# ShittyWizard/DiplomJourney

Hardware: NVIDIA B200
Metric: candidate rollouts/s (MPC inner loop) (higher is better)
Workload: dtype f32

## Files before the change

### diplomjourney_b200/build.py

```python
from __future__ import annotations

import hashlib
import os
import shutil
import subprocess
import sys

HERE = os.path.dirname(os.path.abspath(__file__))
CSRC = os.path.join(HERE, "csrc")
LIB = os.environ.get("MPCB_LIB") or os.path.join(HERE, "lib", "libmpcb200.so")
SOURCES = ["mpcb_kernels.cu", "mpcb_loop.cu", "mpcb_api.cu", "mpcb_nccl.cu"]
HEADERS = ["mpcb_types.cuh", "mpcb_bounds.cuh", "mpcb_exact.cuh", "mpcb_handle.cuh", "mpcb_events.cuh", "mpcb_noise.cuh", "mpcb_pcg64.cuh", "mpcb_screen.cuh", os.path.join("..", "..", "include", "mpcb200.h")]
NVCC_FLAGS = [
    "-gencode", "arch=compute_100a,code=sm_100a", "-O3", "-lineinfo", "-std=c++17",
    "-Xcompiler", "-fPIC", "-Xcompiler", "-fvisibility=hidden", "--shared",
]


def _nvcc() -> str:
    for cand in (os.environ.get("NVCC"), shutil.which("nvcc"), "/usr/local/cuda/bin/nvcc"):
        if cand and os.path.exists(cand):
            return cand
    raise RuntimeError("nvcc not found: the CUDA library cannot be built (there is no CPU fallback)")


def source_hash() -> str:
    h = hashlib.sha256(" ".join(NVCC_FLAGS).encode())
    for name in SOURCES + HEADERS:
        with open(os.path.join(CSRC, name), "rb") as f:
            h.update(name.encode() + b"\0" + f.read())
    return h.hexdigest()


def needs_build(lib: str | None = None) -> bool:
    lib = lib or LIB
    try:
        with open(lib + ".srchash") as f:
            return not os.path.exists(lib) or f.read().strip() != source_hash()
    except OSError:
        return True


def build_library(force: bool = False, verbose: bool = False, extra_flags=(), out: str | None = None) -> str:
    out = out or LIB
    if not force and out == LIB and (os.environ.get("MPCB_LIB") or not needs_build()):
        if not os.path.exists(LIB):
            raise RuntimeError(f"MPCB_LIB={LIB} does not exist")
        return LIB
    os.makedirs(os.path.dirname(out), exist_ok=True)
    cmd = [_nvcc()] + NVCC_FLAGS + list(extra_flags) + (["-Xptxas", "-v"] if verbose else []) + \
          [os.path.join(CSRC, s) for s in SOURCES] + ["-o", out, "-ldl"]
    r = subprocess.run(cmd, capture_output=True, text=True)
    if r.returncode != 0:
        raise RuntimeError("nvcc failed:\n" + r.stdout + r.stderr)
    if not extra_flags:
        with open(out + ".srchash", "w") as f:
            f.write(source_hash() + "\n")
    if verbose:
        print(r.stderr)
    return out


if __name__ == "__main__":
    print(build_library(force="--force" in sys.argv, verbose="-v" in sys.argv))
```

### diplomjourney_b200/csrc/mpcb_api.cu

```cuda
#include "../../include/mpcb200.h"
#include "mpcb_types.cuh"
#include "mpcb_bounds.cuh"
#include "mpcb_handle.cuh"
#include "mpcb_noise.cuh"
#include "mpcb_pcg64.cuh"

#include <algorithm>
#include <cmath>
#include <cstdarg>
#include <cstdio>
#include <cstring>
#include <string>
#include <vector>

namespace mpcb {
cudaError_t launch_prep(cudaStream_t, long long, const double *, const double *, const double *, const double *,
                        const uint8_t *, int, int, int, double, double, double, SolveParams *);
cudaError_t launch_pass(cudaStream_t, const LaunchArgs &, const RowPairs &, int pass, bool prefix, int sms);
cudaError_t launch_reduce_compact(cudaStream_t, const LaunchArgs &, double *, unsigned *, unsigned *, int sms);
cudaError_t launch_reduce_compact_wide(cudaStream_t, const LaunchArgs &, double *, unsigned *, unsigned *, void *scratch,
                                       int sms, int *launches);
cudaError_t launch_probe(cudaStream_t, const LaunchArgs &, int sms);
cudaError_t launch_tilecut(cudaStream_t, const LaunchArgs &, unsigned long long g_begin, unsigned long long g_end,
                           unsigned long long *list, unsigned *count, unsigned long long list_cap);
cudaError_t launch_frontier_expand(cudaStream_t, const LaunchArgs &, int k, const unsigned long long *src,
                                   const unsigned *src_count, unsigned long long *dst, unsigned *dst_count,
                                   unsigned *overflow, int sms);
cudaError_t launch_tilewalk_fallback(cudaStream_t, const LaunchArgs &, unsigned long long all_tiles, int sms);
cudaError_t launch_cand_resolve(cudaStream_t, const LaunchArgs &, int sms);
cudaError_t launch_refine_scan(cudaStream_t, const LaunchArgs &, int sms);
cudaError_t launch_finalize(cudaStream_t, const LaunchArgs &, double *, long long *, double *, double *);
cudaError_t launch_dump(cudaStream_t, const LaunchArgs &, bool prefix, double *jrel, int sms);
cudaError_t launch_held_loop(cudaStream_t, const LoopArgs &, int sms);
cudaError_t launch_rng_seed(cudaStream_t, long long N, const unsigned *keys, int key_len, unsigned *rng_state);
cudaError_t launch_pcg64_seed(cudaStream_t, long long N, const unsigned *entropy, int ent_len, int ent_stride,
                              const unsigned *spawn, int spawn_len, unsigned long long *pcg_state);
cudaError_t launch_held_small(cudaStream_t, const SmallArgs &);
cudaError_t launch_full_apply(cudaStream_t, const FullLoopArgs &);
cudaError_t launch_held_windows(cudaStream_t, const WindowArgs &, int sms);
cudaError_t launch_split_ub_min(cudaStream_t, const LaunchArgs &, const unsigned long long *all, int nranks);
cudaError_t launch_split_pack(cudaStream_t, const LaunchArgs &, SplitRec *mine);
cudaError_t launch_split_pick(cudaStream_t, const LaunchArgs &, const SplitRec *all, int nranks);
bool nccl_available();
int nccl_comm_info(void *comm, int *nranks, int *rank);
int nccl_allgather_bytes(void *comm, const void *send, void *recv, size_t bytes, cudaStream_t st);
}

using namespace mpcb;

namespace {

int fail(mpcb_handle *h, int code, const char *fmt, ...) {
    char buf[512];
    va_list ap;
    va_start(ap, fmt);
// ... 102 lines not shown
    std::vector<float2> c32(S), c32s(S);
    double vmin_grid = v[0];
    for (int i = 1; i < nv; ++i) vmin_grid = std::min(vmin_grid, v[i]);
    const double v_slow = vmin_grid > v_min ? vmin_grid : v_min;
    double smax = 0, dphimax = 0, smin = INFINITY;
    for (int iv = 0; iv < nv; ++iv)
        for (int ib = 0; ib < nb; ++ib) {
            const int c = iv * nb + ib;
            for (int variant = 0; variant < 2; ++variant) {
                const double vc = variant ? v_slow : v[iv];
                const double dphi = (vc / L) * std::tan(beta[ib]) * delta_t;
                const double s = vc * delta_t;
                const double cd = std::cos(dphi), sd = std::sin(dphi);
                smax = std::max(smax, std::fabs(s));
                smin = std::min(smin, s);
                dphimax = std::max(dphimax, std::fabs(dphi));
                if (variant == 0) {
                    t64[c] = make_double4(cd, sd, s, dphi);
                    vt[c] = vc;
                    l32[c] = make_float4((float)(s * cd), (float)(s * sd), (float)(s * s),
                                         (float)(3.16227766016837952 * dphi));
                    c32[c] = make_float2((float)dphi, (float)s);
                } else {
                    t64s[c] = make_double4(cd, sd, s, dphi);
                    vts[c] = vc;
                    c32s[c] = make_float2((float)dphi, (float)s);
                }
            }
        }
    std::vector<float4> t32(S);
    for (int c = 0; c < S; ++c) t32[c] = make_float4((float)t64[c].x, (float)t64[c].y, (float)t64[c].z, (float)t64[c].w);
    CK(h->tab32.ensure(sizeof(float4) * S));
    CK(h->tab64.ensure(sizeof(double4) * S)); CK(h->tab64_slow.ensure(sizeof(double4) * S));
    CK(h->vtab.ensure(sizeof(double) * S)); CK(h->vtab_slow.ensure(sizeof(double) * S));
    CK(h->beta.ensure(sizeof(double) * nb));
    const int npairs = (S + 1) / 2;
    std::vector<float4> l32p(2 * (size_t)npairs);
    for (int m = 0; m < npairs; ++m) {
        const float4 x = l32[2 * m], y = l32[std::min(2 * m + 1, S - 1)];
        l32p[2 * m] = make_float4(x.x, y.x, x.y, y.y);
        l32p[2 * m + 1] = make_float4(x.z, y.z, x.w, y.w);
    }
    const int ppr = (nb + 1) / 2;
    const bool rows_fit = 2LL * nv * ppr <= kLeafChunk;
    std::vector<float4> l32r(rows_fit ? 2 * (size_t)nv * ppr : 0);
    if (rows_fit)
        for (int iv = 0; iv < nv; ++iv)
            for (int m = 0; m < ppr; ++m) {
                const float4 x = l32[iv * nb + 2 * m], y = l32[iv * nb + std::min(2 * m + 1, nb - 1)];
                l32r[2 * ((size_t)iv * ppr + m)] = make_float4(x.x, y.x, x.y, y.y);
                l32r[2 * ((size_t)iv * ppr + m) + 1] = make_float4(x.z, y.z, x.w, y.w);
                h->row_ab.ab[iv * ppr + m] = l32r[2 * ((size_t)iv * ppr + m)];
            }
    CK(h->leaf32r.ensure(sizeof(float4) * std::max<size_t>(l32r.size(), 1)));
    CK(h->leaf32.ensure(sizeof(float4) * S));
    CK(h->leaf32p.ensure(sizeof(float4) * 2 * npairs));
    CK(h->ctl32.ensure(sizeof(float2) * S)); CK(h->ctl32_slow.ensure(sizeof(float2) * S));
    CK(cudaMemcpyAsync(h->tab64.p, t64.data(), sizeof(double4) * S, cudaMemcpyHostToDevice, h->stream));
    CK(cudaMemcpyAsync(h->tab32.p, t32.data(), sizeof(float4) * S, cudaMemcpyHostToDevice, h->stream));
    CK(cudaMemcpyAsync(h->tab64_slow.p, t64s.data(), sizeof(double4) * S, cudaMemcpyHostToDevice, h->stream));
    CK(cudaMemcpyAsync(h->vtab.p, vt.data(), sizeof(double) * S, cudaMemcpyHostToDevice, h->stream));
    CK(cudaMemcpyAsync(h->vtab_slow.p, vts.data(), sizeof(double) * S, cudaMemcpyHostToDevice, h->stream));
    CK(cudaMemcpyAsync(h->beta.p, beta, sizeof(double) * nb, cudaMemcpyHostToDevice, h->stream));
    CK(cudaMemcpyAsync(h->leaf32.p, l32.data(), sizeof(float4) * S, cudaMemcpyHostToDevice, h->stream));
    CK(cudaMemcpyAsync(h->leaf32p.p, l32p.data(), sizeof(float4) * 2 * npairs, cudaMemcpyHostToDevice, h->stream));
    if (rows_fit) CK(cudaMemcpyAsync(h->leaf32r.p, l32r.data(), sizeof(float4) * l32r.size(), cudaMemcpyHostToDevice, h->stream));
    CK(cudaMemcpyAsync(h->ctl32.p, c32.data(), sizeof(float2) * S, cudaMemcpyHostToDevice, h->stream));
    CK(cudaMemcpyAsync(h->ctl32_slow.p, c32s.data(), sizeof(float2) * S, cudaMemcpyHostToDevice, h->stream));
    GridTables &g = h->g;
    g.tab64 = h->tab64.as<double4>(); g.vtab = h->vtab.as<double>();
    g.tab32 = h->tab32.as<float4>();
    g.tab64_slow = h->tab64_slow.as<double4>(); g.vtab_slow = h->vtab_slow.as<double>();
    g.beta = h->beta.as<double>();
    g.leaf32 = h->leaf32.as<float4>();
    g.leaf32p = h->leaf32p.as<float4>();
    g.leaf32r = rows_fit ? h->leaf32r.as<float4>() : nullptr;
    g.nv = nv; g.ppr = rows_fit ? ppr : 0;
    g.ctl32 = h->ctl32.as<float2>(); g.ctl32_slow = h->ctl32_slow.as<float2>();
    g.S = S; g.nb = nb; g.dt = delta_t; g.smax = smax; g.dphimax = dphimax; g.smin = smin;
    g.sbox = ScreenBox{l32[0].x, l32[0].x, l32[0].y, l32[0].y, l32[0].w, l32[0].w};
    for (int c = 1; c < S; ++c) {
        g.sbox.amin = std::min(g.sbox.amin, l32[c].x); g.sbox.amax = std::max(g.sbox.amax, l32[c].x);
        g.sbox.bmin = std::min(g.sbox.bmin, l32[c].y); g.sbox.bmax = std::max(g.sbox.bmax, l32[c].y);
        g.sbox.gmin = std::min(g.sbox.gmin, l32[c].w); g.sbox.gmax = std::max(g.sbox.gmax, l32[c].w);
    }
    h->tables_ready = true;
    return MPCB_OK;
}


extern "C" {

int mpcb_version(void) { return 100; }

int mpcb_device_count(void) {
    int n = 0;
    if (cudaGetDeviceCount(&n) != cudaSuccess) return 0;
    return n;
}

int mpcb_create(int device_ordinal, mpcb_handle **out) {
    if (!out) return MPCB_ERR_INVALID;
    *out = nullptr;
    int n = 0;
    if (cudaGetDeviceCount(&n) != cudaSuccess || n <= 0) return MPCB_ERR_NO_DEVICE;
    if (device_ordinal < 0 || device_ordinal >= n) return MPCB_ERR_INVALID;
    mpcb_handle *h = new mpcb_handle_s();
    h->device = device_ordinal;
    if (cudaSetDevice(device_ordinal) != cudaSuccess ||
        cudaStreamCreateWithFlags(&h->stream, cudaStreamNonBlocking) != cudaSuccess) {
        delete h;
        return MPCB_ERR_CUDA;
    }
    cudaDeviceGetAttribute(&h->sms, cudaDevAttrMultiProcessorCount, device_ordinal);
    *out = h;
    return MPCB_OK;
}

int mpcb_destroy(mpcb_handle *h) {
    if (!h) return MPCB_OK;
    cudaSetDevice(h->device);
    cudaStreamSynchronize(h->stream);
    for (DevBuf *b : {&h->tab64, &h->tab32, &h->vtab, &h->tab64_slow, &h->vtab_slow, &h->beta, &h->leaf32, &h->leaf32p, &h->leaf32r, &h->ctl32,
                      &h->ctl32_slow, &h->sp, &h->segmin, &h->worklist, &h->misc, &h->tau, &h->bestJ, &h->bestIdx,
                      &h->lock, &h->ub, &h->tile_list, &h->reduce_scratch, &h->in_state, &h->in_target, &h->in_origin, &h->in_thr, &h->in_flags, &h->out_cost,
                      &h->out_index, &h->out_traj, &h->out_ctl, &h->dump_rec, &h->dump_j, &h->loop_log, &h->loop_ticks,
                      &h->loop_status, &h->loop_events, &h->loop_final, &h->loop_rng, &h->loop_keys, &h->small_in, &h->small_out, &h->fl_last, &h->fl_k, &h->fl_have, &h->fl_flags,
                      &h->fl_count, &h->nccl_scratch, &h->cand, &h->cand_J, &h->cand_sel, &h->node_list})
        b->release();
    if (h->pin_in) cudaFreeHost(h->pin_in);
    if (h->pin_out) cudaFreeHost(h->pin_out);
    cudaStreamDestroy(h->stream);
    delete h;
    return MPCB_OK;
}

const char *mpcb_last_error(const mpcb_handle *h) { return h ? h->err.c_str() : "null handle"; }
void *mpcb_stream(mpcb_handle *h) { return h ? (void *)h->stream : nullptr; }

int mpcb_sync(mpcb_handle *h) {
    if (!h) return MPCB_ERR_INVALID;
    CK(cudaSetDevice(h->device));
    CK(cudaStreamSynchronize(h->stream));
    return MPCB_OK;
}

int mpcb_set_option(mpcb_handle *h, const char *name, double value) {
    if (!h || !name) return MPCB_ERR_INVALID;
    if (!strcmp(name, "tol_scale")) h->tol_scale = value;
    else if (!strcmp(name, "algo")) h->algo = (int)value;
    else if (!strcmp(name, "refine")) h->refine = value != 0.0;
    else if (!strcmp(name, "small_path")) h->small_path = value != 0.0;
    else if (!strcmp(name, "zero_copy")) h->zero_copy = value != 0.0;
    else if (!strcmp(name, "candidate_list")) {
        if (value == -1.0) { h->cand_cap = 1u << 20; h->cand_auto = true; return MPCB_OK; }
        if (!(value >= 0.0 && value <= (double)(1u << 26))) return fail(h, MPCB_ERR_INVALID, "candidate_list out of range [0, 2^26] (or -1)");
        h->cand_cap = (unsigned)value; h->cand_auto = false;
    }
    else if (!strcmp(name, "node_list")) {
        if (!(value >= 0.0 && value <= (double)(1u << 24))) return fail(h, MPCB_ERR_INVALID, "node_list out of range [0, 2^24]");
        h->node_cap = (unsigned)value;
    }
    else if (!strcmp(name, "prune")) h->prune = value != 0.0;
    else if (!strcmp(name, "dump_direct")) h->dump_direct = value != 0.0;
    else if (!strcmp(name, "screen")) {
        if (value != 0.0 && value != 1.0 && value != 2.0) return fail(h, MPCB_ERR_INVALID, "screen must be 0, 1 or 2");
        h->screen = (int)value;
    }
    else if (!strcmp(name, "prefilter")) h->prefilter = value != 0.0;
    else if (!strcmp(name, "subtree_cut")) {
        if (value != 0.0 && value != 1.0 && value != 2.0 && value != 3.0) return fail(h, MPCB_ERR_INVALID, "subtree_cut must be 0, 1, 2 or 3");
        h->subtree_cut = (int)value;
    }
    else if (!strcmp(name, "frontier_cap")) {
        if (!(value >= 1.0 && value <= (double)(1ULL << 28))) return fail(h, MPCB_ERR_INVALID, "frontier_cap out of range [1, 2^28]");
        h->frontier_cap = (unsigned long long)value;
// ... 901 lines not shown
```

### diplomjourney_b200/csrc/mpcb_kernels.cu

```cuda
#include <type_traits>

#include "mpcb_types.cuh"
#include "mpcb_bounds.cuh"
#include "mpcb_exact.cuh"

#ifndef MPCB_UNROLL2
#define MPCB_UNROLL2 8
#endif
#ifndef MPCB_UNROLL4
#define MPCB_UNROLL4 2
#endif
#ifndef MPCB_PN_CTA2
#define MPCB_PN_CTA2 512
#endif
#ifndef MPCB_UNROLL_ROWS
#define MPCB_UNROLL_ROWS 4
#endif
#ifndef MPCB_UNROLL_DIST
#define MPCB_UNROLL_DIST 7
#endif
#ifndef MPCB_UNROLL
#define MPCB_UNROLL 8
#endif

#include <cfloat>
#include <cmath>

namespace mpcb {

__device__ __forceinline__ float sqrt_approx(float x) {
    float y;
    asm("sqrt.approx.ftz.f32 %0, %1;" : "=f"(y) : "f"(x));
    return y;
}
__device__ __forceinline__ float rcp_approx(float x) {
    float y;
    asm("rcp.approx.ftz.f32 %0, %1;" : "=f"(y) : "f"(x));
    return y;
}
__device__ __forceinline__ double4 ldg_d4(const double4 *p) {
    const double2 *q = reinterpret_cast<const double2 *>(p);
    double2 a = __ldg(q), b = __ldg(q + 1);
    return make_double4(a.x, a.y, b.x, b.y);
}
__device__ __forceinline__ double warp_min(double v) {
#pragma unroll
    for (int o = 16; o > 0; o >>= 1) v = fmin(v, __shfl_xor_sync(0xffffffffu, v, o));
    return v;
}
__device__ __forceinline__ unsigned long long ordered_key(double v) {
    unsigned long long b = (unsigned long long)__double_as_longlong(v);
    return b ^ ((b >> 63) ? ~0ULL : 0x8000000000000000ULL);
}
__device__ __forceinline__ double ordered_value(unsigned long long k) {
    if (k == ~0ULL) return INFINITY;
    unsigned long long b = (k >> 63) ? (k ^ 0x8000000000000000ULL) : ~k;
    return __longlong_as_double((long long)b);
}
__device__ __forceinline__ void lex_min(double &J, long long &j, double oJ, long long oj) {
    if (oj >= 0 && (j < 0 || oJ < J || (oJ == J && oj < j))) { J = oJ; j = oj; }
}

struct ParentRegs {
    float u, w;
    float u2, w2;
    float D2, Dp;
    float nu, nw;
    float e2, h2;
    float eh, nhh;
    float u2s, w2s, D2s;
};

// ... 306 lines not shown
            const float2 q = __ffma2_rn(NU[k], A, __ffma2_rn(NW[k], B, E[k]));
            float2 t = __ffma2_rn(make_float2(-q.x, -q.y), q, C[k]);
            if (HEAD) { const float2 gg = __fadd2_rn(G, Hh[k]); t = __ffma2_rn(make_float2(-gg.x, -gg.y), gg, t); }
            const float2 df = __ffma2_rn(t, t, ndd);
            m[k] = fmaxf(m[k], fmaxf(df.x, df.y));
        }
    }
#pragma unroll
    for (int k = 0; k < NPT; ++k) mx[k] = m[k];
}

template <bool HEAD, int NPT>
__device__ __forceinline__ void prefix_screen_loop_rows(const float4 *__restrict__ tab, int nv, int ppr,
                                                        const ParentRegs (&p)[NPT], const float (&cn)[NPT],
                                                        float (&mx)[NPT]) {
    float2 U[NPT], W[NPT], NU[NPT], NW[NPT], E[NPT], Hh[NPT], C[NPT];
    float nD[NPT], m[NPT];
#pragma unroll
    for (int k = 0; k < NPT; ++k) {
        U[k] = make_float2(-p[k].u2s, -p[k].u2s); W[k] = make_float2(-p[k].w2s, -p[k].w2s);
        nD[k] = -p[k].D2s;
        NU[k] = make_float2(p[k].nu, p[k].nu); NW[k] = make_float2(p[k].nw, p[k].nw);
        E[k] = make_float2(p[k].eh, p[k].eh); Hh[k] = make_float2(p[k].nhh, p[k].nhh);
        C[k] = make_float2(cn[k], cn[k]);
        m[k] = -INFINITY;
    }
    constexpr int kUnroll = NPT == 2 ? MPCB_UNROLL_ROWS : MPCB_UNROLL4;
    for (int iv = 0; iv < nv; ++iv) {
        const float4 *__restrict__ row = tab + 2 * iv * ppr;
        const float rv = row[1].x;
        float2 DV[NPT];
#pragma unroll
        for (int k = 0; k < NPT; ++k) { const float d = __fmaf_rn(-kWd2f, rv, nD[k]); DV[k] = make_float2(d, d); }
#pragma unroll kUnroll
        for (int i = 0; i < ppr; ++i) {
            const float4 t0 = row[2 * i];
            const float2 G = reinterpret_cast<const float2 *>(row + 2 * i + 1)[1];
            const float2 A = make_float2(t0.x, t0.y), B = make_float2(t0.z, t0.w);
#pragma unroll
            for (int k = 0; k < NPT; ++k) {
                const float2 ndd = __ffma2_rn(U[k], A, __ffma2_rn(W[k], B, DV[k]));
                const float2 q = __ffma2_rn(NU[k], A, __ffma2_rn(NW[k], B, E[k]));
                float2 t = __ffma2_rn(make_float2(-q.x, -q.y), q, C[k]);
                if (HEAD) { const float2 gg = __fadd2_rn(G, Hh[k]); t = __ffma2_rn(make_float2(-gg.x, -gg.y), gg, t); }
                const float2 df = __ffma2_rn(t, t, ndd);
                m[k] = fmaxf(m[k], fmaxf(df.x, df.y));
            }
        }
    }
#pragma unroll
    for (int k = 0; k < NPT; ++k) mx[k] = m[k];
}

template <int NPT>
__device__ __forceinline__ void prefix_dist_loop_rows(const RowPairs &ab, const float4 *__restrict__ tab, int nv, int ppr,
                                                      const ParentRegs (&p)[NPT], float (&mx)[NPT]) {
    float2 U[NPT], W[NPT];
    float nD[NPT], m[NPT];
#pragma unroll
    for (int k = 0; k < NPT; ++k) {
        U[k] = make_float2(-p[k].u2s, -p[k].u2s); W[k] = make_float2(-p[k].w2s, -p[k].w2s);
        nD[k] = -p[k].D2s;
        m[k] = -INFINITY;
    }
    constexpr int kUnroll = MPCB_UNROLL_DIST;
    const float4 *__restrict__ row = tab;
    const float4 *pair = ab.ab;
    for (int iv = 0; iv < nv; ++iv, row += 2 * ppr, pair += ppr) {
        const float rv = row[1].x;
        float2 DV[NPT];
#pragma unroll
        for (int k = 0; k < NPT; ++k) { const float d = __fmaf_rn(-kWd2f, rv, nD[k]); DV[k] = make_float2(d, d); }
#pragma unroll kUnroll
        for (int i = 0; i < ppr; ++i) {
            const float4 t0 = pair[i];
            const float2 A = make_float2(t0.x, t0.y), B = make_float2(t0.z, t0.w);
#pragma unroll
            for (int k = 0; k < NPT; ++k) {
                const float2 ndd = __ffma2_rn(U[k], A, __ffma2_rn(W[k], B, DV[k]));
                m[k] = fmaxf(m[k], fmaxf(ndd.x, ndd.y));
            }
        }
    }
#pragma unroll
    for (int k = 0; k < NPT; ++k) mx[k] = m[k];
}

template <bool HEAD>
__device__ __forceinline__ float prefix_min_loop_scalar(const float4 *__restrict__ tab, int npairs, const ParentRegs &pr,
                                                        bool near, bool special, float Lspecial, float best) {
    for (int m = 0; m < npairs; ++m) {
        const float4 t0 = tab[2 * m], t1 = tab[2 * m + 1];
        float L0 = near ? leaf_val<HEAD, true>(t0.x, t0.z, t1.x, t1.z, pr) : leaf_val<HEAD, false>(t0.x, t0.z, t1.x, t1.z, pr);
        float L1 = near ? leaf_val<HEAD, true>(t0.y, t0.w, t1.y, t1.w, pr) : leaf_val<HEAD, false>(t0.y, t0.w, t1.y, t1.w, pr);
        if (special && t1.x == 0.f) L0 = Lspecial;
        if (special && t1.y == 0.f) L1 = Lspecial;
        best = fminf(best, fminf(L0, L1));
    }
    return best;
}

template <int PASS, bool HEAD, bool PRUNE = false, bool QMODE = false>
__global__ void __launch_bounds__((PASS == 1 && !PRUNE) ? kPrefixCta : kThreads, (PASS == 1 && !PRUNE) ? 1 : 4)
prefix_kernel(const LaunchArgs a) {
    static_assert(PASS == 1, "pass 2 of the prefix algorithm is refine_prefix_kernel");
    extern __shared__ float4 s_leaf[];
    const int tid = threadIdx.x;
    const int S = a.g.S;
    const bool single = S <= kLeafChunk;
    const float4 *__restrict__ gtab = PASS == 1 ? a.g.leaf32p : a.g.leaf32;
    auto chunk_f4 = [&](int cn) { return PASS == 1 ? 2 * ((cn + 1) >> 1) : cn; };
    if (single) {
        for (int i = tid; i < chunk_f4(S); i += blockDim.x) s_leaf[i] = __ldg(gtab + i);
        __syncthreads();
    }
    const unsigned groups = blockDim.x / kThreads;
    const unsigned long long qps = (a.tiles_per_solve + groups - 1) / groups;
    constexpr bool qmode = PASS == 1 && PRUNE && QMODE;
    const bool listed = PASS == 1 && PRUNE && !QMODE && a.tile_list != nullptr;
    if (PASS == 1 && PRUNE && gate_closed(a)) return;
    const unsigned qrounds = (unsigned)((S + kThreads - 1) / kThreads);
    if (qmode && blockIdx.x == 0 && tid == 0) atomicAdd(a.counters + 2, a.counters[3]);
    const unsigned long long nwork =
        qmode ? (unsigned long long)min(*a.q_count, a.q_cap) * qrounds
        : listed ? (unsigned long long)(*a.tile_count)
                 : PASS == 1 ? (unsigned long long)a.N * qps : (unsigned long long)(*a.work_count) * a.tps;
    unsigned long long cut_acc = 0;
// ... 329 lines not shown
prefixn_kernel(const LaunchArgs a, const __grid_constant__ RowPairs ab) {
    extern __shared__ float4 s_leaf[];
    constexpr int kCta = prefixn_cta(NPT);
    const int tid = threadIdx.x;
    const int S = a.g.S;
    const bool rows = SCREEN && a.g.ppr > 0;
    const bool single = rows || S <= kLeafChunk;
    const float4 *__restrict__ gtab = rows ? a.g.leaf32r : a.g.leaf32p;
    auto chunk_f4 = [&](int cn) { return 2 * ((cn + 1) >> 1); };
    if (single) {
        for (int i = tid; i < (rows ? 2 * a.g.nv * a.g.ppr : chunk_f4(S)); i += blockDim.x) s_leaf[i] = __ldg(gtab + i);
        __syncthreads();
    }
    constexpr unsigned groups = kCta * NPT / kThreads;
    static_assert(kCta * NPT % kThreads == 0, "a work item is a whole number of tiles");
    const unsigned long long qps = (a.tiles_per_solve + groups - 1) / groups;
    const unsigned long long nwork = (unsigned long long)a.N * qps;
    unsigned long long stage2_acc = 0;
    for (unsigned long long w = blockIdx.x; w < nwork; w += gridDim.x) {
        const long long n = (long long)(w / qps);
        const unsigned long long tile0 = (w - (unsigned long long)n * qps) * groups;
        const SolveParams &P = a.sp[n];
        if (__reduce_or_sync(0xffffffffu, (unsigned)P.flags & kFlagSkip)) continue;
        const bool origin_case = (P.flags & kFlagStartIsOrigin) != 0;
        auto slot = [&](int k, unsigned long long &p, unsigned &sg) {
            const unsigned node = tid + k * kCta;
            const unsigned long long tile = tile0 + node / kThreads;
            p = a.u_begin + tile * kThreads + (node % kThreads);
            sg = (unsigned)((unsigned long long)n * a.segs_per_solve + (a.tps == 1 ? tile : tile / a.tps));
            return tile < a.tiles_per_solve && p < a.u_end;
        };
        double ubw = INFINITY;
        if (SCREEN) ubw = ordered_value(*(volatile unsigned long long *)(a.ub + n)) + P.tol1;
        const int npairs_rows = a.g.nv * a.g.ppr;
        double v[NPT];
        double vhit = INFINITY;
#pragma unroll
        for (int k = 0; k < NPT; ++k) v[k] = INFINITY;
        if constexpr (SCREEN == 2) {
            ParentRegs s1[NPT] = {};
            float tmax[NPT];
            unsigned staged = 0, direct = 0;
#pragma unroll
            for (int k = 0; k < NPT; ++k) {
                unsigned long long p;
                unsigned sg;
                tmax[k] = 0.f;
                if (!slot(k, p, sg)) continue;
                ParentRegs q;
                bool nr, um;
                double bd;
                parent_setup(a, P, p, q, nr, um, nullptr, &bd);
                if (nr || (origin_case && um)) { direct |= 1u << k; continue; }
                staged |= 1u << k;
                s1[k].u2s = q.u2s; s1[k].w2s = q.w2s; s1[k].D2s = q.D2s;
                tmax[k] = screen_stage1_tmax(a.g.sbox, HEAD, __double2float_ru(ubw - bd), q.nu, q.nw, q.eh, q.nhh);
            }
            unsigned rare = direct;
            if (__reduce_or_sync(0xffffffffu, staged)) {
                float mdd[NPT];
                prefix_dist_loop_rows<NPT>(ab, s_leaf, a.g.nv, a.g.ppr, s1, mdd);
#pragma unroll
                for (int k = 0; k < NPT; ++k)
                    if (((staged >> k) & 1u) && screen_stage1_pass(tmax[k], mdd[k])) { rare |= 1u << k; ++stage2_acc; }
            }
            for (unsigned m = rare; m; m &= m - 1) {
                const int k = __ffs(m) - 1;
                unsigned long long p;
                unsigned sg;
                slot(k, p, sg);
                ParentRegs pr;
                bool near, unmoved;
                double bd;
                double base = parent_setup(a, P, p, pr, near, unmoved, nullptr, &bd);
                float best = INFINITY;
                if ((direct >> k) & 1u) {
                    const float Ls = (float)(P.special - 0.25 * (double)pr.e2 * (double)pr.e2);
                    best = prefix_min_loop_scalar<HEAD>(s_leaf, npairs_rows, pr, near, origin_case && unmoved, Ls, best);
                } else {
                    base = bd;
                    const ParentRegs one[1] = {pr};
                    const float cn[1] = {__double2float_ru(ubw - bd)};
                    float mx[1];
                    prefix_screen_loop_rows<HEAD, 1>(s_leaf, a.g.nv, a.g.ppr, one, cn, mx);
                    if (mx[0] > 0.f) {
                        best = prefix_min_loop_far2<HEAD>(s_leaf, npairs_rows, pr, best);
                        vhit = fmin(vhit, base + (double)best);
                    }
                }
#pragma unroll
                for (int j = 0; j < NPT; ++j)
                    if (j == k) v[j] = base + (double)best;
            }
        } else {
            ParentRegs pr[NPT] = {};
            bool near[NPT], special[NPT], active[NPT];
            double base[NPT];
            float best[NPT], Lspecial[NPT], cn[NPT];
            bool all = true;
#pragma unroll
            for (int k = 0; k < NPT; ++k) {
                unsigned long long p;
                unsigned sg;
                active[k] = slot(k, p, sg);
                bool unmoved = false;
                near[k] = false; base[k] = 0.0; best[k] = INFINITY;
                double base_direct = 0.0;
                if (active[k]) base[k] = parent_setup(a, P, p, pr[k], near[k], unmoved, nullptr, &base_direct);
                special[k] = active[k] && origin_case && unmoved;
                if (!(near[k] || special[k])) base[k] = base_direct;
                Lspecial[k] = (float)(P.special - 0.25 * (double)pr[k].e2 * (double)pr[k].e2);
                cn[k] = SCREEN ? __double2float_ru(ubw - base_direct) : 0.f;
                all = all && active[k] && !near[k] && !special[k];
            }
// ... 1000 lines not shown
```

### diplomjourney_b200/csrc/mpcb_types.cuh

```cuda
#pragma once
#include <cmath>
#include <cstdint>
#include <cuda_runtime.h>

#include "../../include/mpcb200.h"
#include "mpcb_screen.cuh"

namespace mpcb {

#ifndef MPCB_THREADS
#define MPCB_THREADS 256
#endif
constexpr int kThreads = MPCB_THREADS;
constexpr int kPrefixCta = 1024;
constexpr int kMaxH = 8;
constexpr int kLeafChunk = 1024;

constexpr double kWd = 10000.0;

#ifdef __CUDACC__
#define MPCB_HD __host__ __device__ __forceinline__
#define MPCB_HD_NOINLINE __host__ __device__ __noinline__
#else
#define MPCB_HD inline
// ... 38 lines not shown
        unsigned long long t = __umul64hi(m, n);
#else
        unsigned long long t = (unsigned long long)(((unsigned __int128)m * n) >> 64);
#endif
        return (t + ((n - t) >> sh1)) >> sh2;
    }
};

struct FastDiv32 {
    unsigned m, d, sh1, sh2;
    MPCB_HD unsigned div(unsigned n) const {
#ifdef __CUDA_ARCH__
        unsigned t = __umulhi(m, n);
#else
        unsigned t = (unsigned)(((unsigned long long)m * n) >> 32);
#endif
        return (t + ((n - t) >> sh1)) >> sh2;
    }
};

inline void fastdiv32_init(FastDiv32 &f, unsigned long long d64) {
    unsigned d = (unsigned)d64;
    f.d = d;
    if (d <= 1) { f.m = 0; f.sh1 = 0; f.sh2 = 0; return; }
    unsigned l = 0;
    while ((l < 32) && ((1ULL << l) < d)) ++l;
    f.m = (unsigned)((((1ULL << l) - d) << 32) / d) + 1u;
    f.sh1 = 1; f.sh2 = l - 1;
}

inline void fastdiv_init(FastDiv64 &f, unsigned long long d) {
    f.d = d;
    if (d <= 1) { f.m = 0; f.sh1 = 0; f.sh2 = 0; return; }
    unsigned l = 0;
    while ((l < 64) && ((1ULL << l) < d)) ++l;
    unsigned __int128 num = ((unsigned __int128)1 << 64) * (((unsigned __int128)1 << l) - d);
    f.m = (unsigned long long)(num / d) + 1ULL;
    f.sh1 = 1; f.sh2 = l - 1;
}

constexpr int kLeafPerThread = 8;

struct GridTables {
    const double4 *tab64;
    const double  *vtab;
    const float4  *tab32;
    const double4 *tab64_slow;
    const double  *vtab_slow;
    const double  *beta;
    const float4 *leaf32;
    const float4 *leaf32p;
    const float4 *leaf32r;
    int nv, ppr;
    const float2 *ctl32;
    const float2 *ctl32_slow;
    int S, nb;
    double dt;
    double smax, dphimax;
    double smin;
    ScreenBox sbox;
};

constexpr int kRowPairCap = kLeafChunk / 2;
struct RowPairs { float4 ab[kRowPairCap]; };

struct __align__(16) SolveParams {
    double xs, ys, phi0;
    double xt, yt;
    double ox, oy;
    double theta;
    double lineA, lineB, lineC, line_norm;
    double threshold;
    double u0, w0, d0;
    double e0, nx0, ny0;
    double hp0;
    double wl, wh;
    double inv_wl;
    double Kbase;
    double tol;
    double tol1;
    double special;
    int flags;
    int pad;
    float pf[12];
};
constexpr int kFlagSlow = 1, kFlagStartIsOrigin = 2, kFlagNear = 4, kFlagSkip = 8;

struct __align__(8) Candidate { long long j; double jrel; int n; int pad; };

struct __align__(16) RefineNode {
    float u, w, u2, w2, D2, Dp, nu, nw, e2, h2;
    float thr, Lspecial;
    double base;
    unsigned long long p;
    int n;
    unsigned flags;
};

struct LaunchArgs {
    GridTables g;
    const SolveParams *sp;
    FastDiv64 fd[kMaxH];
    FastDiv32 fd32[kMaxH];
    FastDiv64 fd_tiles, fd_S;
    int idx32;
    int node32;
    unsigned step_digits[kMaxH];
    int lw_smem;
    unsigned tile_units;
    int mode, H, cost_kind, refine;
    long long N;
    unsigned long long u_begin, u_end;
    unsigned long long tiles_per_solve, segs_per_solve, total_segs;
// ... 85 lines not shown
```

### diplomjourney_b200/csrc/mpcb_handle.cuh

```cuda
#pragma once
#include <string>
#include <vector>

#include "mpcb_types.cuh"

namespace mpcb {

struct DevBuf {
    void *p = nullptr;
    size_t cap = 0;
    cudaError_t ensure(size_t bytes) {
        if (bytes <= cap) return cudaSuccess;
        if (p) cudaFree(p);
        p = nullptr; cap = 0;
        size_t want = bytes + bytes / 4 + 256;
        cudaError_t e = cudaMalloc(&p, want);
        if (e == cudaSuccess) cap = want;
        return e;
    }
    void release() { if (p) cudaFree(p); p = nullptr; cap = 0; }
    template <typename T> T *as() { return reinterpret_cast<T *>(p); }
};

constexpr unsigned long long kSegCap = 1ULL << 22;
constexpr unsigned long long kTileBatch = 1ULL << 23;
constexpr unsigned long long kWideReduceSegs = 1ULL << 15;
constexpr unsigned long long kFrontierCap = 1ULL << 22;

}

struct mpcb_handle_s {
    int device = 0, sms = 148;
    cudaStream_t stream = nullptr;
    std::string err;
    bool have_grid = false, tables_ready = false;
    std::vector<double> hv, hb;
    double L = 0, delta_t = 0, v_min = 0, v_slow = 0;
    mpcb::GridTables g{};
    mpcb::DevBuf tab64, tab32, vtab, tab64_slow, vtab_slow, beta, leaf32, leaf32p, leaf32r, ctl32, ctl32_slow;
    mpcb::RowPairs row_ab{};
    double tol_scale = 1.0;
    int algo = MPCB_ALGO_AUTO;
    int refine = 1;
    int small_path = 1;
    int zero_copy = 1;
    int dump_direct = 0;
    int npt = 4;
    unsigned long long frontier_cap = mpcb::kFrontierCap;
    int subtree_cut = 2;
    int screen = 2;
    int prefilter = 1;
    int prune = 1;
    mpcb::DevBuf sp, segmin, worklist, misc, tau, bestJ, bestIdx, lock, ub, tile_list, reduce_scratch;
    mpcb::DevBuf in_state, in_target, in_origin, in_thr, in_flags, out_cost, out_index, out_traj, out_ctl, dump_rec, dump_j;
    mpcb::DevBuf cand, cand_J, cand_sel;
    mpcb::DevBuf node_list;
    unsigned node_cap = 1u << 15;
    unsigned cand_cap = 1u << 20;
    bool cand_auto = true;
    mpcb::DevBuf nccl_scratch;
    mpcb::DevBuf loop_log, loop_ticks, loop_status, loop_events, loop_final, loop_rng, loop_keys, loop_pcg, loop_pcg_spawn, small_in, small_out, fl_last, fl_k, fl_have, fl_flags, fl_count;
    void *pin_in = nullptr, *pin_out = nullptr;
    size_t pin_in_cap = 0, pin_out_cap = 0;
    mpcb_stats stats{};
};
```

### diplomjourney_b200/csrc/mpcb_screen.cuh

```cuda
#pragma once
#include <cmath>

#if defined(__CUDACC__)
#define MPCB_SCR_HD __host__ __device__ __forceinline__
#else
#define MPCB_SCR_HD inline
#endif

namespace mpcb {

struct ScreenBox {
    float amin, amax, bmin, bmax, gmin, gmax;
};

MPCB_SCR_HD float scr_fma(float a, float b, float c) {
#if defined(__CUDA_ARCH__)
    return __fmaf_rn(a, b, c);
#else
    return std::fma(a, b, c);
#endif
}

MPCB_SCR_HD float scr_add(float a, float b) {
#if defined(__CUDA_ARCH__)
    return __fadd_rn(a, b);
#else
    return a + b;
#endif
}

MPCB_SCR_HD float scr_near0(float lo, float hi) { return lo > 0.f ? lo : (hi < 0.f ? hi : 0.f); }
MPCB_SCR_HD float scr_far0(float lo, float hi) { return std::fabs(lo) > std::fabs(hi) ? lo : hi; }

MPCB_SCR_HD void screen_q_range(const ScreenBox &bx, float nu, float nw, float eh, float &lo, float &hi) {
    const float ilo = scr_fma(nw, nw >= 0.f ? bx.bmin : bx.bmax, eh), ihi = scr_fma(nw, nw >= 0.f ? bx.bmax : bx.bmin, eh);
    lo = scr_fma(nu, nu >= 0.f ? bx.amin : bx.amax, ilo);
    hi = scr_fma(nu, nu >= 0.f ? bx.amax : bx.amin, ihi);
}
MPCB_SCR_HD void screen_g_range(const ScreenBox &bx, float nhh, float &lo, float &hi) {
    lo = scr_add(bx.gmin, nhh);
    hi = scr_add(bx.gmax, nhh);
}

MPCB_SCR_HD void screen_t_range(const ScreenBox &bx, bool head, float cn, float nu, float nw, float eh, float nhh,
                                float &tlo, float &thi) {
    float qlo, qhi;
    screen_q_range(bx, nu, nw, eh, qlo, qhi);
    const float qn = scr_near0(qlo, qhi), qf = scr_far0(qlo, qhi);
    thi = scr_fma(-qn, qn, cn);
    tlo = scr_fma(-qf, qf, cn);
    if (head) {
        float glo, ghi;
        screen_g_range(bx, nhh, glo, ghi);
        const float gn = scr_near0(glo, ghi), gf = scr_far0(glo, ghi);
        thi = scr_fma(-gn, gn, thi);
        tlo = scr_fma(-gf, gf, tlo);
    }
}

MPCB_SCR_HD float screen_stage1_tmax(const ScreenBox &bx, bool head, float cn, float nu, float nw, float eh, float nhh) {
    float tlo, thi;
    screen_t_range(bx, head, cn, nu, nw, eh, nhh, tlo, thi);
    const float ah = std::fabs(thi), al = std::fabs(tlo);
    return (ah != ah || al != al) ? ah + al : (ah > al ? ah : al);
}

MPCB_SCR_HD bool screen_stage1_pass(float tmax, float maxndd) { return !(scr_fma(tmax, tmax, maxndd) <= 0.f); }

}
```

Measured before the change: 9499 billion.

## Fold mirror-symmetric steering grid in prefix distance screening loop

Detects on the host when the leaf grid is mirror-symmetric in its second component (x equal, y negated across the steering axis). In that case it packs only half the steering classes with absolute y values and runs the distance screen on the folded rows using |w|, so each row needs roughly half the inner iterations. The fold unroll factor is set separately. This relies on the max over mirrored pairs being equal to the max using absolute values; grids that are not symmetric take the old path.

```diff
diff --git a/diplomjourney_b200/build.py b/diplomjourney_b200/build.py
--- a/diplomjourney_b200/build.py
+++ b/diplomjourney_b200/build.py
@@ -10,7 +10,7 @@
 CSRC = os.path.join(HERE, "csrc")
 LIB = os.environ.get("MPCB_LIB") or os.path.join(HERE, "lib", "libmpcb200.so")
 SOURCES = ["mpcb_kernels.cu", "mpcb_loop.cu", "mpcb_api.cu", "mpcb_nccl.cu"]
-HEADERS = ["mpcb_types.cuh", "mpcb_bounds.cuh", "mpcb_exact.cuh", "mpcb_handle.cuh", "mpcb_events.cuh", "mpcb_noise.cuh", "mpcb_pcg64.cuh", "mpcb_screen.cuh", os.path.join("..", "..", "include", "mpcb200.h")]
+HEADERS = ["mpcb_types.cuh", "mpcb_bounds.cuh", "mpcb_exact.cuh", "mpcb_handle.cuh", "mpcb_events.cuh", "mpcb_noise.cuh", "mpcb_pcg64.cuh", "mpcb_screen.cuh", "mpcb_fold.cuh", os.path.join("..", "..", "include", "mpcb200.h")]
 NVCC_FLAGS = [
     "-gencode", "arch=compute_100a,code=sm_100a", "-O3", "-lineinfo", "-std=c++17",
     "-Xcompiler", "-fPIC", "-Xcompiler", "-fvisibility=hidden", "--shared",
diff --git a/diplomjourney_b200/csrc/mpcb_api.cu b/diplomjourney_b200/csrc/mpcb_api.cu
--- a/diplomjourney_b200/csrc/mpcb_api.cu
+++ b/diplomjourney_b200/csrc/mpcb_api.cu
@@ -1,6 +1,7 @@
 #include "../../include/mpcb200.h"
 #include "mpcb_types.cuh"
 #include "mpcb_bounds.cuh"
+#include "mpcb_fold.cuh"
 #include "mpcb_handle.cuh"
 #include "mpcb_noise.cuh"
 #include "mpcb_pcg64.cuh"
@@ -209,6 +210,8 @@
                 l32r[2 * ((size_t)iv * ppr + m) + 1] = make_float4(x.z, y.z, x.w, y.w);
                 h->row_ab.ab[iv * ppr + m] = l32r[2 * ((size_t)iv * ppr + m)];
             }
+    const bool folds = rows_fit && grid_folds(&l32[0].x, nv, nb);
+    if (folds) fold_pack(&l32[0].x, nv, nb, &h->row_ab.ab[0].x);
     CK(h->leaf32r.ensure(sizeof(float4) * std::max<size_t>(l32r.size(), 1)));
     CK(h->leaf32.ensure(sizeof(float4) * S));
     CK(h->leaf32p.ensure(sizeof(float4) * 2 * npairs));
@@ -233,6 +236,7 @@
     g.leaf32p = h->leaf32p.as<float4>();
     g.leaf32r = rows_fit ? h->leaf32r.as<float4>() : nullptr;
     g.nv = nv; g.ppr = rows_fit ? ppr : 0;
+    g.fpr = folds ? fold_entries_per_row(nb) : 0;
     g.ctl32 = h->ctl32.as<float2>(); g.ctl32_slow = h->ctl32_slow.as<float2>();
     g.S = S; g.nb = nb; g.dt = delta_t; g.smax = smax; g.dphimax = dphimax; g.smin = smin;
     g.sbox = ScreenBox{l32[0].x, l32[0].x, l32[0].y, l32[0].y, l32[0].w, l32[0].w};
diff --git a/diplomjourney_b200/csrc/mpcb_fold.cuh b/diplomjourney_b200/csrc/mpcb_fold.cuh
--- /dev/null
+++ b/diplomjourney_b200/csrc/mpcb_fold.cuh
@@ -0,0 +1,29 @@
+#pragma once
+#include <cmath>
+
+namespace mpcb {
+
+inline int fold_classes(int nb) { return (nb + 1) / 2; }
+inline int fold_entries_per_row(int nb) { return (fold_classes(nb) + 1) / 2; }
+
+inline bool grid_folds(const float *leaf, int nv, int nb) {
+    for (int iv = 0; iv < nv; ++iv)
+        for (int ib = 0; ib < fold_classes(nb); ++ib) {
+            const float *x = leaf + 4 * ((long long)iv * nb + ib), *y = leaf + 4 * ((long long)iv * nb + nb - 1 - ib);
+            if (!(x[0] == y[0] && x[1] == -y[1])) return false;
+        }
+    return true;
+}
+
+inline void fold_pack(const float *leaf, int nv, int nb, float *out) {
+    const int nc = fold_classes(nb), fpr = fold_entries_per_row(nb);
+    for (int iv = 0; iv < nv; ++iv)
+        for (int m = 0; m < fpr; ++m) {
+            const float *x = leaf + 4 * ((long long)iv * nb + 2 * m);
+            const float *y = leaf + 4 * ((long long)iv * nb + (2 * m + 1 < nc ? 2 * m + 1 : nc - 1));
+            float *o = out + 4 * ((long long)iv * fpr + m);
+            o[0] = x[0]; o[1] = y[0]; o[2] = std::fabs(x[1]); o[3] = std::fabs(y[1]);
+        }
+}
+
+}
diff --git a/diplomjourney_b200/csrc/mpcb_kernels.cu b/diplomjourney_b200/csrc/mpcb_kernels.cu
--- a/diplomjourney_b200/csrc/mpcb_kernels.cu
+++ b/diplomjourney_b200/csrc/mpcb_kernels.cu
@@ -18,6 +18,9 @@
 #endif
 #ifndef MPCB_UNROLL_DIST
 #define MPCB_UNROLL_DIST 7
+#endif
+#ifndef MPCB_UNROLL_FOLD
+#define MPCB_UNROLL_FOLD 11
 #endif
 #ifndef MPCB_UNROLL
 #define MPCB_UNROLL 8
@@ -430,27 +433,28 @@
     for (int k = 0; k < NPT; ++k) mx[k] = m[k];
 }
 
-template <int NPT>
+template <int NPT, bool FOLD>
 __device__ __forceinline__ void prefix_dist_loop_rows(const RowPairs &ab, const float4 *__restrict__ tab, int nv, int ppr,
-                                                      const ParentRegs (&p)[NPT], float (&mx)[NPT]) {
+                                                      int epr, const ParentRegs (&p)[NPT], float (&mx)[NPT]) {
     float2 U[NPT], W[NPT];
     float nD[NPT], m[NPT];
 #pragma unroll
     for (int k = 0; k < NPT; ++k) {
-        U[k] = make_float2(-p[k].u2s, -p[k].u2s); W[k] = make_float2(-p[k].w2s, -p[k].w2s);
+        const float w = FOLD ? fabsf(p[k].w2s) : -p[k].w2s;
+        U[k] = make_float2(-p[k].u2s, -p[k].u2s); W[k] = make_float2(w, w);
         nD[k] = -p[k].D2s;
         m[k] = -INFINITY;
     }
-    constexpr int kUnroll = MPCB_UNROLL_DIST;
+    constexpr int kUnroll = FOLD ? MPCB_UNROLL_FOLD : MPCB_UNROLL_DIST;
     const float4 *__restrict__ row = tab;
     const float4 *pair = ab.ab;
-    for (int iv = 0; iv < nv; ++iv, row += 2 * ppr, pair += ppr) {
+    for (int iv = 0; iv < nv; ++iv, row += 2 * ppr, pair += epr) {
         const float rv = row[1].x;
         float2 DV[NPT];
 #pragma unroll
         for (int k = 0; k < NPT; ++k) { const float d = __fmaf_rn(-kWd2f, rv, nD[k]); DV[k] = make_float2(d, d); }
 #pragma unroll kUnroll
-        for (int i = 0; i < ppr; ++i) {
+        for (int i = 0; i < epr; ++i) {
             const float4 t0 = pair[i];
             const float2 A = make_float2(t0.x, t0.y), B = make_float2(t0.z, t0.w);
 #pragma unroll
@@ -893,7 +897,8 @@
             unsigned rare = direct;
             if (__reduce_or_sync(0xffffffffu, staged)) {
                 float mdd[NPT];
-                prefix_dist_loop_rows<NPT>(ab, s_leaf, a.g.nv, a.g.ppr, s1, mdd);
+                if (a.g.fpr) prefix_dist_loop_rows<NPT, true>(ab, s_leaf, a.g.nv, a.g.ppr, a.g.fpr, s1, mdd);
+                else prefix_dist_loop_rows<NPT, false>(ab, s_leaf, a.g.nv, a.g.ppr, a.g.ppr, s1, mdd);
 #pragma unroll
                 for (int k = 0; k < NPT; ++k)
                     if (((staged >> k) & 1u) && screen_stage1_pass(tmax[k], mdd[k])) { rare |= 1u << k; ++stage2_acc; }
diff --git a/diplomjourney_b200/csrc/mpcb_types.cuh b/diplomjourney_b200/csrc/mpcb_types.cuh
--- a/diplomjourney_b200/csrc/mpcb_types.cuh
+++ b/diplomjourney_b200/csrc/mpcb_types.cuh
@@ -114,6 +114,7 @@
     const float4 *leaf32p;
     const float4 *leaf32r;
     int nv, ppr;
+    int fpr;
     const float2 *ctl32;
     const float2 *ctl32_slow;
     int S, nb;
```

Result: faster. 13350 billion, median of 6 (+40.5%).

## Add arc-based stage-1 screening bound to prune parents before staging

Applied to the files above, without the earlier changes.

Precomputes, for each velocity row, an arc of the reachable heading directions plus error bounds on the host and uploads them as a per-row table. In the stage-1 screen, each parent computes a rigorous upper bound over all rows using that arc geometry and skips staging when the bound shows no candidate can beat the current upper bound. The aim is to cut how many parents go through the expensive stage-1 leaf evaluation. The cost is a per-parent loop over nv rows in double precision and extra global loads, which could outweigh the savings if pruning is weak.

```diff
diff --git a/diplomjourney_b200/csrc/mpcb_api.cu b/diplomjourney_b200/csrc/mpcb_api.cu
--- a/diplomjourney_b200/csrc/mpcb_api.cu
+++ b/diplomjourney_b200/csrc/mpcb_api.cu
@@ -224,7 +224,26 @@
     if (rows_fit) CK(cudaMemcpyAsync(h->leaf32r.p, l32r.data(), sizeof(float4) * l32r.size(), cudaMemcpyHostToDevice, h->stream));
     CK(cudaMemcpyAsync(h->ctl32.p, c32.data(), sizeof(float2) * S, cudaMemcpyHostToDevice, h->stream));
     CK(cudaMemcpyAsync(h->ctl32_slow.p, c32s.data(), sizeof(float2) * S, cudaMemcpyHostToDevice, h->stream));
+    std::vector<ScreenArc> arcs(nv);
+    double arc_eps = 0.0, arc_krmax = 0.0, arc_smax = 0.0;
+    {
+        std::vector<double> dphi(nb);
+        std::vector<float> ra(nb), rb(nb);
+        for (int iv = 0; iv < nv; ++iv) {
+            for (int ib = 0; ib < nb; ++ib) {
+                const int c = iv * nb + ib;
+                dphi[ib] = t64[c].w; ra[ib] = l32[c].x; rb[ib] = l32[c].y;
+            }
+            arc_eps = std::max(arc_eps, screen_row_arc(v[iv] * delta_t, nb, dphi.data(), ra.data(), rb.data(), l32[iv * nb].z, arcs[iv]));
+            arc_krmax = std::max(arc_krmax, arcs[iv].kr);
+            arc_smax = std::max(arc_smax, arcs[iv].s_abs);
+        }
+    }
+    CK(h->arcs.ensure(sizeof(ScreenArc) * nv));
+    CK(cudaMemcpyAsync(h->arcs.p, arcs.data(), sizeof(ScreenArc) * nv, cudaMemcpyHostToDevice, h->stream));
     GridTables &g = h->g;
+    g.arcs = h->arcs.as<ScreenArc>();
+    g.arc_eps = arc_eps; g.arc_krmax = arc_krmax; g.arc_smax = arc_smax;
     g.tab64 = h->tab64.as<double4>(); g.vtab = h->vtab.as<double>();
     g.tab32 = h->tab32.as<float4>();
     g.tab64_slow = h->tab64_slow.as<double4>(); g.vtab_slow = h->vtab_slow.as<double>();
@@ -278,7 +297,7 @@
     if (!h) return MPCB_OK;
     cudaSetDevice(h->device);
     cudaStreamSynchronize(h->stream);
-    for (DevBuf *b : {&h->tab64, &h->tab32, &h->vtab, &h->tab64_slow, &h->vtab_slow, &h->beta, &h->leaf32, &h->leaf32p, &h->leaf32r, &h->ctl32,
+    for (DevBuf *b : {&h->tab64, &h->tab32, &h->vtab, &h->tab64_slow, &h->vtab_slow, &h->beta, &h->leaf32, &h->leaf32p, &h->leaf32r, &h->arcs, &h->ctl32,
                       &h->ctl32_slow, &h->sp, &h->segmin, &h->worklist, &h->misc, &h->tau, &h->bestJ, &h->bestIdx,
                       &h->lock, &h->ub, &h->tile_list, &h->reduce_scratch, &h->in_state, &h->in_target, &h->in_origin, &h->in_thr, &h->in_flags, &h->out_cost,
                       &h->out_index, &h->out_traj, &h->out_ctl, &h->dump_rec, &h->dump_j, &h->loop_log, &h->loop_ticks,
diff --git a/diplomjourney_b200/csrc/mpcb_handle.cuh b/diplomjourney_b200/csrc/mpcb_handle.cuh
--- a/diplomjourney_b200/csrc/mpcb_handle.cuh
+++ b/diplomjourney_b200/csrc/mpcb_handle.cuh
@@ -37,7 +37,7 @@
     std::vector<double> hv, hb;
     double L = 0, delta_t = 0, v_min = 0, v_slow = 0;
     mpcb::GridTables g{};
-    mpcb::DevBuf tab64, tab32, vtab, tab64_slow, vtab_slow, beta, leaf32, leaf32p, leaf32r, ctl32, ctl32_slow;
+    mpcb::DevBuf tab64, tab32, vtab, tab64_slow, vtab_slow, beta, leaf32, leaf32p, leaf32r, arcs, ctl32, ctl32_slow;
     mpcb::RowPairs row_ab{};
     double tol_scale = 1.0;
     int algo = MPCB_ALGO_AUTO;
diff --git a/diplomjourney_b200/csrc/mpcb_kernels.cu b/diplomjourney_b200/csrc/mpcb_kernels.cu
--- a/diplomjourney_b200/csrc/mpcb_kernels.cu
+++ b/diplomjourney_b200/csrc/mpcb_kernels.cu
@@ -886,9 +886,12 @@
                 double bd;
                 parent_setup(a, P, p, q, nr, um, nullptr, &bd);
                 if (nr || (origin_case && um)) { direct |= 1u << k; continue; }
+                tmax[k] = screen_stage1_tmax(a.g.sbox, HEAD, __double2float_ru(ubw - bd), q.nu, q.nw, q.eh, q.nhh);
+                const float ub1 = screen_stage1_arc_bound(a.g.arcs, a.g.nv, a.g.arc_eps, a.g.arc_krmax, a.g.arc_smax,
+                                                          q.u2s, q.w2s, q.D2s);
+                if (scr_fma(tmax[k], tmax[k], ub1) <= 0.f) continue;
                 staged |= 1u << k;
                 s1[k].u2s = q.u2s; s1[k].w2s = q.w2s; s1[k].D2s = q.D2s;
-                tmax[k] = screen_stage1_tmax(a.g.sbox, HEAD, __double2float_ru(ubw - bd), q.nu, q.nw, q.eh, q.nhh);
             }
             unsigned rare = direct;
             if (__reduce_or_sync(0xffffffffu, staged)) {
diff --git a/diplomjourney_b200/csrc/mpcb_screen.cuh b/diplomjourney_b200/csrc/mpcb_screen.cuh
--- a/diplomjourney_b200/csrc/mpcb_screen.cuh
+++ b/diplomjourney_b200/csrc/mpcb_screen.cuh
@@ -67,4 +67,49 @@
 
 MPCB_SCR_HD bool screen_stage1_pass(float tmax, float maxndd) { return !(scr_fma(tmax, tmax, maxndd) <= 0.f); }
 
+struct ScreenArc {
+    double s_abs, lo_x, lo_y, kr;
+    double hi_x, hi_y, wide, pad;
+};
+
+inline double screen_row_arc(double s, int nb, const double *dphi, const float *a, const float *b, float r, ScreenArc &arc) {
+    const double sg = s < 0.0 ? -1.0 : 1.0;
+    double lo = INFINITY, hi = -INFINITY, eps = 0.0;
+    for (int ib = 0; ib < nb; ++ib) {
+        lo = std::fmin(lo, dphi[ib]); hi = std::fmax(hi, dphi[ib]);
+        eps = std::fmax(eps, std::fmax(std::fabs((double)a[ib] - s * std::cos(dphi[ib])),
+                                       std::fabs((double)b[ib] - s * std::sin(dphi[ib]))));
+    }
+    arc.s_abs = std::fabs(s);
+    arc.lo_x = sg * std::cos(lo); arc.lo_y = sg * std::sin(lo);
+    arc.hi_x = sg * std::cos(hi); arc.hi_y = sg * std::sin(hi);
+    arc.kr = 1.0e8 * (double)r;
+    arc.wide = hi - lo > 1.5707963267948966 ? 1.0 : 0.0;
+    arc.pad = 0.0;
+    return eps * (1.0 + 0x1p-20) + 0x1p-1000;
 }
+
+MPCB_SCR_HD float screen_stage1_arc_bound(const ScreenArc *arcs, int nv, double eps, double krmax, double smax,
+                                          float u2s, float w2s, float D2s) {
+    const double U = -(double)u2s, W = -(double)w2s, D = D2s;
+    const double M = std::fabs(D) + krmax + (smax + eps) * (std::fabs(U) + std::fabs(W));
+    if (!(M < INFINITY)) return NAN;
+    const double R = std::sqrt(U * U + W * W), tol = 0x1p-30 * R;
+    double best = -INFINITY;
+    for (int v = 0; v < nv; ++v) {
+        const ScreenArc &c = arcs[v];
+        const bool inside = c.wide != 0.0 || (c.lo_x * W - c.lo_y * U >= -tol && U * c.hi_y - W * c.hi_x >= -tol);
+        const double m = inside ? R : std::fmax(U * c.lo_x + W * c.lo_y, U * c.hi_x + W * c.hi_y);
+        best = std::fmax(best, c.s_abs * m - c.kr);
+    }
+    const double b = best - D + (std::fabs(U) + std::fabs(W)) * eps + 3.0 * 0x1p-24 * M * (1.0 + 0x1p-20) + 0x1p-40 * M + 0x1p-140;
+#if defined(__CUDA_ARCH__)
+    return __double2float_ru(b);
+#else
+    float f = (float)b;
+    if ((double)f < b) f = std::nextafter(f, INFINITY);
+    return f;
+#endif
+}
+
+}
diff --git a/diplomjourney_b200/csrc/mpcb_types.cuh b/diplomjourney_b200/csrc/mpcb_types.cuh
--- a/diplomjourney_b200/csrc/mpcb_types.cuh
+++ b/diplomjourney_b200/csrc/mpcb_types.cuh
@@ -121,6 +121,8 @@
     double smax, dphimax;
     double smin;
     ScreenBox sbox;
+    const ScreenArc *arcs;
+    double arc_eps, arc_krmax, arc_smax;
 };
 
 constexpr int kRowPairCap = kLeafChunk / 2;
```

Result: faster. 9492 billion before, 9681 billion after (median of 6 runs) (+2.0%).
